# TravisWheelerLab/HAVAC

Measured on AMD Instinct MI355X. Metric: GCUPS (billion SSV cells/s); hit-list bit-exact vs softSsv, higher is better.
Workload: dtype i16

## Files before the change

havac_amd/csrc/ssv_kernels.hip.h:

```cpp
#pragma once
#include <hip/hip_runtime.h>
#include <stdint.h>
#include <utility>

namespace havac {

constexpr int kDiagsPerLane = 32;
constexpr int kRegs = kDiagsPerLane / 2;
constexpr int kTileDiags = 64 * kDiagsPerLane;
constexpr int kChunkRows = 32;
constexpr int kChunkPairs = kChunkRows / 2;
#ifndef HAVAC_BATCH
#define HAVAC_BATCH 8
#endif
#ifndef HAVAC_WAVES_PER_SIMD
#define HAVAC_WAVES_PER_SIMD 6
#endif
#ifndef HAVAC_WAVES_PER_BLOCK
#define HAVAC_WAVES_PER_BLOCK 4
#endif
constexpr int kWavesPerBlock = HAVAC_WAVES_PER_BLOCK;
constexpr int kModelSlack = 40;
constexpr uint32_t kScoreZero = 0x80008000u;
constexpr uint32_t kCrossedBits = 0x00010001u;
constexpr uint32_t kOutsideReset = 0x80008000u;
constexpr uint32_t kOutsideNeutral = 0u;
constexpr uint32_t kPadRow = 0u;
constexpr int kMaxRowCuts = 32;
constexpr int kMaxWalkRounds = 8;
constexpr int kWindowSteps = 4;

constexpr int kPairStride = 17 * 8;
constexpr uint32_t kOutsideCode = 16 * 8;
constexpr int kTableBytes = 2304;
constexpr int kHitStage = 128;
constexpr int kTailSlots = 128;
constexpr int kTicketStride = 16;
constexpr int kTicketCounters = 8;

__device__ __forceinline__ uint64_t hit_key(uint32_t row, uint64_t column, uint32_t row_bits) {
    const uint32_t seg = (uint32_t)(column >> 12) / 3u;
    const uint32_t in_seg = (uint32_t)column - seg * 12288u;
    return ((uint64_t)seg << (14 + row_bits)) | ((uint64_t)row << 14) | in_seg;
}

__device__ __forceinline__ uint64_t key_to_record(uint64_t key, uint32_t row_bits) {
    uint64_t in_seg = key & 0x3fffull;
    uint64_t row = (key >> 14) & ((1ull << row_bits) - 1ull);
    uint64_t seg = key >> (14 + row_bits);
    return in_seg | (seg << 14) | (row << 40);
}
__device__ __forceinline__ uint64_t record_to_key(uint64_t rec, uint32_t row_bits) {
    uint64_t in_seg = rec & 0x3fffull;
    uint64_t seg = (rec >> 14) & 0x3ffffffull;
    uint64_t row = rec >> 40;
    return (seg << (14 + row_bits)) | (row << 14) | in_seg;
}

__device__ __forceinline__ uint32_t padded_model_row(const uint32_t* __restrict__ phmm_rows, uint32_t nrows, uint32_t i) {
    return (i >= 1 && i <= nrows) ? phmm_rows[i - 1] : kPadRow;
}

__global__ void ssv_prepare_model(const int8_t* __restrict__ phmm, uint32_t nrows, uint32_t* __restrict__ rows, uint32_t nwords,
                                  uint32_t nrows_padded, uint32_t* __restrict__ flags, uint32_t nflagwords ,
                                  unsigned long long* __restrict__ hit_count, uint32_t* __restrict__ control, uint32_t ncontrol,
                                  uint32_t* __restrict__ handoff, uint32_t nhandoff) {
    const uint32_t* const phmm_rows = reinterpret_cast<const uint32_t*>(phmm);
    const uint32_t i = blockIdx.x * blockDim.x + threadIdx.x;
    if (i == 0) *hit_count = 0ull;
    if (i < ncontrol) control[i] = 0u;
    for (uint32_t k = i; k < nhandoff; k += gridDim.x * blockDim.x) handoff[k] = 0u;
    if (i < nwords) rows[i] = padded_model_row(phmm_rows, nrows, i);
    if (nflagwords == 0) return;
    const uint32_t chunk = i;
    const uint32_t p0 = chunk * kChunkRows;
    if (chunk / 4 >= nflagwords) return;
    uint32_t bits = 0;
    if (p0 < nrows_padded + kChunkRows) {
        int lowest[kChunkRows + 3];
#pragma unroll
        for (int k = 0; k < kChunkRows + 3; k++) {
            const uint32_t r = padded_model_row(phmm_rows, nrows, p0 + 1 + k);
            int m = 0;
#pragma unroll
            for (int a = 0; a < 4; a++) m = min(m, (int)(int8_t)(r >> (8 * a)));
            lowest[k] = m;
        }
#pragma unroll
        for (int q = 0; q < kChunkRows / kWindowSteps; q++) {
            const int high = lowest[4 * q] + lowest[4 * q + 1] + lowest[4 * q + 2], low = lowest[4 * q + 1] + lowest[4 * q + 2] + lowest[4 * q + 3];
            if (high >= -255 && low >= -255) bits |= 1u << q;
        }
    }
    reinterpret_cast<uint8_t*>(flags)[chunk] = (uint8_t)bits;
}

__global__ void ssv_pack_chars(const uint8_t* __restrict__ chars, uint64_t first_column, uint64_t nchars,
                               uint64_t ncolumns, uint32_t* __restrict__ packed) {
    const uint64_t word = first_column / 16 + (uint64_t)blockIdx.x * blockDim.x + threadIdx.x;
    const uint64_t column = word * 16;
    if (column >= ncolumns) return;
    uint32_t out = 0;
    if (column + 16 <= nchars) {
        const uint4 v = *reinterpret_cast<const uint4*>(chars + (column - first_column));
        const uint32_t w[4] = {v.x, v.y, v.z, v.w};
#pragma unroll
        for (int k = 0; k < 4; k++) {
            uint32_t t = (w[k] >> 1) & 0x03030303u;
            t ^= (t >> 1) & 0x01010101u;
            const uint32_t byte = (t | (t >> 6) | (t >> 12) | (t >> 18)) & 0xffu;
            out |= byte << (8 * k);
        }
    } else {
        for (int i = 0; i < 16; i++) {
            if (column + i >= nchars) break;
            uint32_t t = (chars[column - first_column + i] >> 1) & 3u;
            t ^= t >> 1;
            out |= t << (2 * i);
        }
    }
    packed[word] = out;
}

__global__ void ssv_patch_symbols(const uint64_t* __restrict__ columns, const uint8_t* __restrict__ symbols,
                                  uint64_t npatches, uint32_t* __restrict__ packed) {
    const uint64_t i = (uint64_t)blockIdx.x * blockDim.x + threadIdx.x;
    if (i >= npatches) return;
    const uint64_t column = columns[i];
    const uint32_t shift = (uint32_t)(column % 16) * 2;
    atomicAnd(&packed[column / 16], ~(3u << shift));
    atomicOr(&packed[column / 16], (uint32_t)(symbols[i] & 3u) << shift);
}

__global__ void ssv_pack_records(const uint8_t* __restrict__ chars, const uint64_t* __restrict__ out_start,
                                 const uint64_t* __restrict__ src_begin, const uint64_t* __restrict__ len, uint32_t nrecords,
                                 uint64_t layout_end, uint64_t ncolumns, uint32_t* __restrict__ packed, uint8_t* __restrict__ mask) {
    const uint64_t word = (uint64_t)blockIdx.x * blockDim.x + threadIdx.x;
    const uint64_t col0 = word * 16;
    if (col0 >= ncolumns) return;
    uint32_t lo = 0, hi = nrecords;
    while (lo < hi) {
        const uint32_t mid = (lo + hi) / 2;
        if (out_start[mid] <= col0) lo = mid + 1; else hi = mid;
    }
    uint32_t j = lo ? lo - 1 : 0;
    uint32_t out = 0, bits = 0;
    for (int i = 0; i < 16; i++) {
        const uint64_t col = col0 + i;
        while (j + 1 < nrecords && out_start[j + 1] <= col) j++;
        if (nrecords && col >= out_start[j]) {
            const uint64_t off = col - out_start[j];
            if (off < len[j]) {
                const uint32_t ch = chars[src_begin[j] + off] | 0x20u;
                const uint32_t code = ch == 'a' ? 0u : ch == 'c' ? 1u : ch == 'g' ? 2u : 3u;
                out |= code << (2 * i);
            }
            const uint64_t behind = out_start[j] + len[j];
            if ((i & 1) == 0 && col == behind + (behind & 1)) bits |= 1u << (i / 2);
        }
        if ((i & 1) == 0 && col >= layout_end) bits |= 1u << (i / 2);
    }
    packed[word] = out;
    mask[word] = (uint8_t)bits;
}

__global__ void ssv_reverse_strand(uint32_t* __restrict__ packed, uint64_t nf, const uint64_t* __restrict__ starts,
                                   const uint64_t* __restrict__ residues, uint32_t nrecords) {
    const uint64_t word = (uint64_t)blockIdx.x * blockDim.x + threadIdx.x;
    const uint64_t col0 = word * 16;
    if (col0 >= nf) return;
    auto symbol = [&](uint64_t col) -> uint32_t { return (packed[col / 16] >> (2 * (col % 16))) & 3u; };
    uint32_t lo = 0, hi = nrecords;
    while (lo < hi) {
        const uint32_t mid = (lo + hi) / 2;
        if (starts[mid] <= col0) lo = mid + 1; else hi = mid;
    }
    uint32_t j = lo ? lo - 1 : 0;
    uint32_t out = 0;
    for (int i = 0; i < 16; i++) {
        const uint64_t col = col0 + i;
        while (j + 1 < nrecords && starts[j + 1] <= col) j++;
        uint32_t code = symbol(col);
        if (nrecords && col >= starts[j] && col - starts[j] < residues[j])
            code = 3u - symbol(starts[j] + residues[j] - 1 - (col - starts[j]));
        out |= code << (2 * i);
    }
    packed[(nf + col0) / 16] = out;
}

typedef short short2v __attribute__((ext_vector_type(2)));
typedef uint32_t u32x2 __attribute__((ext_vector_type(2)));
typedef const __attribute__((address_space(3))) u32x2* lds_words_t;
typedef __attribute__((address_space(3))) u32x2* lds_words_out_t;

struct __attribute__((aligned(128))) WaveLds {
    uint8_t table[kTableBytes];
    uint64_t stage[kHitStage];
};

struct CellRecord {
    uint8_t prev;
    int8_t match;
    uint8_t score;
    uint8_t hit;
    uint8_t symbol;
    uint8_t pending;
    uint8_t zero;
    uint8_t written;
};

struct SsvRare {
    uint64_t* hits;
    unsigned long long* hit_count;
    uint64_t hit_capacity;
    int64_t col_begin;
    uint64_t col_span;
    const uint32_t* abort_flag;
    const uint16_t* pair_mask;
    uint32_t* tickets;
    uint32_t* block_flags;
    uint32_t* block_state;
    uint32_t* fault;
    uint32_t row_bits;
    int64_t first_diag; uint32_t tile_begin, ntiles;
    int64_t col_end;
    uint32_t parts_log2;
    uint32_t part_begin[9];
    uint32_t tiles_per_item;
    uint32_t single_tiles;
    uint32_t walk_slots, walk_rounds, walk_len[kMaxWalkRounds], walk_base[kMaxWalkRounds];
    uint32_t half_tail;
    uint32_t split_units;
    uint32_t nrow_blocks;
    uint32_t ncuts, uniform_rows;
    uint32_t row_cut[kMaxRowCuts + 1];
    uint64_t* tails; uint32_t* tail_counts;
    struct CellRecord* cells; int64_t cell_col0; uint32_t cell_row0, cell_rows, cell_cols;
};
typedef const __attribute__((address_space(4))) SsvRare* rare_args_t;
__device__ __forceinline__ rare_args_t rare_args() {
    rare_args_t p = (rare_args_t)__builtin_amdgcn_kernarg_segment_ptr();
    asm volatile("" : "+s"(p));
    return p;
}

struct HitSink {
    uint64_t* stage;
};

__device__ __forceinline__ uint64_t staged_to_key(uint64_t staged_record, uint32_t row_bits) {
    return hit_key((uint32_t)(staged_record >> 40), staged_record & ((1ull << 40) - 1ull), row_bits);
}

__device__ __forceinline__ uint32_t flush_hits(const HitSink& sink, const rare_args_t rare, uint32_t staged) {
    if (staged == 0) return 0;
    const uint32_t lane = __lane_id();
    uint64_t* const hits = rare->hits;
    const uint64_t capacity = rare->hit_capacity;
    const uint32_t row_bits = rare->row_bits;
    __builtin_amdgcn_fence(__ATOMIC_ACQ_REL, "wavefront");
    unsigned long long base = 0;
    if (lane == 0) base = atomicAdd(rare->hit_count, (unsigned long long)staged);
    const uint32_t lo = __builtin_amdgcn_readfirstlane((uint32_t)base);
    const uint32_t hi = __builtin_amdgcn_readfirstlane((uint32_t)(base >> 32));
    base = ((unsigned long long)hi << 32) | lo;
    for (uint32_t i = lane; i < staged; i += 64) {
        const unsigned long long idx = base + i;
        if (idx < capacity) hits[idx] = staged_to_key(sink.stage[i], row_bits);
    }
    __builtin_amdgcn_fence(__ATOMIC_ACQ_REL, "wavefront");
    return 0;
}

__device__ __noinline__ uint32_t flush_full(const HitSink sink, const rare_args_t rare, uint32_t staged) {
    return flush_hits(sink, rare, __builtin_amdgcn_readfirstlane(staged));
}

__device__ __forceinline__ int32_t scalar_sat_add(int32_t a, int32_t b) {
    const int32_t saturated = (b >> 31) ^ INT32_MAX;
    int32_t d;
    asm("s_add_i32 %0, %1, %2\n\ts_cselect_b32 %0, %3, %0" : "=&s"(d) : "s"(a), "s"(b), "s"(saturated) : "scc");
    return d;
}

struct ShardColumns { rare_args_t rare; int64_t begin; uint64_t span; };
__device__ __forceinline__ uint32_t emit_cell(const HitSink& sink, const ShardColumns& own, uint32_t staged, uint32_t row, int64_t column) {
    const rare_args_t rare = own.rare;
    if ((uint64_t)(column - own.begin) < own.span) {
        const uint64_t record = ((uint64_t)row << 40) | (uint64_t)column;
        const uint32_t addr = (uint32_t)(uintptr_t)(__attribute__((address_space(3))) uint64_t*)sink.stage + staged * 8;
        uint64_t saved_exec;
        asm volatile("s_mov_b64 %0, exec\n\ts_mov_b64 exec, 1\n\tds_write_b64 %1, %2\n\ts_mov_b64 exec, %0"
                     : "=&s"(saved_exec) : "v"(addr), "v"(record) : "memory");
        staged++;
        if (staged == kHitStage) staged = flush_full(sink, rare, staged);
    }
    return staged;
}

template <int P>
__device__ __forceinline__ u32x2 match_words(uint32_t code_addr, int extra = 0) {
    return *(lds_words_t)(uintptr_t)(code_addr + P * kPairStride + extra);
}
template <bool Resident>
__device__ __forceinline__ constexpr int slid_offset(int entry_index) { return Resident && entry_index < 16 ? kTableBytes : 0; }

__device__ __forceinline__ uint32_t opaque_uniform(uint32_t x) {
    x = __builtin_amdgcn_readfirstlane(x);
    asm("" : "+s"(x));
    return x;
}
__device__ __forceinline__ uint32_t fresh_uniform(uint32_t x) { asm volatile("" : "+s"(x)); return x; }
__device__ __forceinline__ int32_t clamp_to_4096(int64_t v) {
    const int32_t hi = (int32_t)opaque_uniform((uint32_t)((uint64_t)v >> 32));
    const uint32_t lo = opaque_uniform((uint32_t)v);
    return hi < 0 ? 0 : ((hi > 0 || lo > 4096u) ? 4096 : (int32_t)lo);
}

__device__ __forceinline__ uint32_t fresh_lane() {
    uint32_t lane;
    asm volatile("v_mbcnt_lo_u32_b32 %0, -1, 0\n\tv_mbcnt_hi_u32_b32 %0, -1, %0" : "=v"(lane));
    return lane;
}
struct LaneWords { uint32_t sel_second, entries, row_offset, lane8; };
__device__ __forceinline__ LaneWords read_lane_words(uint32_t lds_address) {
    LaneWords w;
    asm volatile("s_mov_b32 m0, %4\n\ts_nop 0\n\t"
                 "ds_read_addtid_b32 %0 offset:0\n\tds_read_addtid_b32 %1 offset:256\n\t"
                 "ds_read_addtid_b32 %2 offset:512\n\tds_read_addtid_b32 %3 offset:768\n\t"
                 "s_waitcnt lgkmcnt(0)"
                 : "=v"(w.sel_second), "=v"(w.entries), "=v"(w.row_offset), "=v"(w.lane8) : "s"(lds_address) : "m0", "memory");
    return w;
}

constexpr uint32_t kFlagSpecial = 2u;
constexpr int kFlagSafeShift = 8;
struct LazySymbols {
    uint32_t even[2], odd[2];
    uint32_t separators;
    uint32_t table_base;
    uint32_t special;
    int32_t valid_lo, valid_hi;
};

__device__ __forceinline__ void prepare_symbols(LazySymbols& z, uint32_t lo, uint32_t hi) {
    z.even[0] = (lo << 3) & 0x78787878u; z.odd[0] = (lo >> 1) & 0x78787878u;
    z.even[1] = (hi << 3) & 0x78787878u; z.odd[1] = (hi >> 1) & 0x78787878u;
}

template <int BYTE>
__device__ __forceinline__ uint32_t or_byte(uint32_t base, uint32_t word) {
    uint32_t out;
    if constexpr (BYTE == 0) asm("v_or_b32_sdwa %0, %1, %2 dst_sel:DWORD dst_unused:UNUSED_PAD src0_sel:DWORD src1_sel:BYTE_0" : "=v"(out) : "s"(base), "v"(word));
    if constexpr (BYTE == 1) asm("v_or_b32_sdwa %0, %1, %2 dst_sel:DWORD dst_unused:UNUSED_PAD src0_sel:DWORD src1_sel:BYTE_1" : "=v"(out) : "s"(base), "v"(word));
    if constexpr (BYTE == 2) asm("v_or_b32_sdwa %0, %1, %2 dst_sel:DWORD dst_unused:UNUSED_PAD src0_sel:DWORD src1_sel:BYTE_2" : "=v"(out) : "s"(base), "v"(word));
    if constexpr (BYTE == 3) asm("v_or_b32_sdwa %0, %1, %2 dst_sel:DWORD dst_unused:UNUSED_PAD src0_sel:DWORD src1_sel:BYTE_3" : "=v"(out) : "s"(base), "v"(word));
    return out;
}

template <int K>
__device__ __forceinline__ void expand_entry(uint32_t (&C)[32], const LazySymbols& z) {
    constexpr int n = K & 7;
    uint32_t entry = or_byte<n / 2>(z.table_base, (n & 1) ? z.odd[K / 8] : z.even[K / 8]);
    if (fresh_uniform(z.special) & kFlagSpecial) {
        const uint32_t lane32 = fresh_lane() * 32u;
        const int32_t q = (int32_t)lane32 + 2 * K;
        if (q < z.valid_lo || q >= z.valid_hi || ((z.separators >> K) & 1u)) entry = z.table_base + kOutsideCode;
    }
    C[16 + K] = entry;
}

template <int Q>
__device__ __forceinline__ void expand_for_window(uint32_t (&C)[32], const LazySymbols& z) {
    if constexpr (Q == 0) {
        expand_entry<0>(C, z);
    } else {
        expand_entry<2 * Q - 1>(C, z);
        expand_entry<2 * Q>(C, z);
    }
}

template <int... K>
__device__ __forceinline__ void expand_all(uint32_t (&C)[32], const LazySymbols& z, std::integer_sequence<int, K...>) {
    (expand_entry<K>(C, z), ...);
}

struct TraceWindow { CellRecord* cells; int64_t col0; uint32_t row0, nrows, ncols; };
__device__ __noinline__ void trace_cells_of_step(TraceWindow win, uint32_t second_of_pair, uint32_t reg, uint32_t t, int64_t wave_diag0,
                                                 uint32_t before, uint32_t mword, uint32_t after, uint32_t code) {
    const int64_t column = wave_diag0 + (int64_t)(32u * __lane_id() + 2u * reg) + (int64_t)t;
    const uint64_t dc = (uint64_t)(column - win.col0);
    const uint8_t symbol = code > 15u ? 0xffu : (uint8_t)(second_of_pair ? code >> 2 : code & 3u);
    for (uint32_t half = 0; half < 2; half++) {
        const uint32_t dr = t - half - win.row0;
        if (dr < win.nrows && dc < (uint64_t)win.ncols) {
            const uint32_t b = (before >> (16 * half)) & 0xffffu, a = (after >> (16 * half)) & 0xffffu;
            CellRecord rec;
            rec.pending = (b & 0xffu) != 0;
            rec.hit = !rec.pending && (a & 0xffu) != 0;
            rec.prev = rec.pending ? 0 : (uint8_t)((b ^ 0x8000u) >> 8);
            rec.score = (rec.pending || rec.hit) ? 0 : (uint8_t)((a ^ 0x8000u) >> 8);
            rec.match = (int8_t)(uint8_t)(mword >> (8 + 16 * half));
            rec.symbol = symbol;
            rec.zero = 0;
            rec.written = 1;
            win.cells[(size_t)dr * win.ncols + (size_t)dc] = rec;
        }
    }
}
__device__ __forceinline__ TraceWindow trace_window() {
    const rare_args_t rare = rare_args();
    return TraceWindow{rare->cells, rare->cell_col0, rare->cell_row0, rare->cell_rows, rare->cell_cols};
}
template <bool SecondOfPair>
__device__ __forceinline__ void trace_step(const TraceWindow& win, uint32_t reg, uint32_t t, int64_t wave_diag0, uint32_t before,
                                           uint32_t mword, uint32_t after, uint32_t entry, uint32_t table_base) {
    trace_cells_of_step(win, SecondOfPair ? 1u : 0u, reg, t, wave_diag0, before, mword, after, (entry - table_base) >> 3);
}

template <int Q, int I>
__device__ __forceinline__ void window_inputs(uint32_t l, const uint32_t (&cur)[kRegs], const uint32_t (&nxt)[kRegs],
                                              const uint32_t (&C)[32], uint32_t& s, uint32_t& now, uint32_t& entry0,
                                              uint32_t& entry1) {
    asm volatile("v_readlane_b32 %0, %4, %8\n\tv_readlane_b32 %1, %5, %8\n\tv_readlane_b32 %2, %6, %8\n\tv_readlane_b32 %3, %7, %8"
                 : "=&s"(s), "=&s"(now), "=&s"(entry0), "=&s"(entry1)
                 : "v"(cur[I]), "v"(nxt[I]), "v"(C[2 * Q + I]), "v"(C[2 * Q + 1 + I]), "s"(l));
}

__device__ __forceinline__ void write_score_lane(uint32_t (&n)[kRegs], uint32_t s, uint32_t l, uint32_t r) {
    static_assert(kRegs == 16, "the asm below names sixteen registers");
    asm volatile("s_mov_b32 m0, %[l]\n\t"
                 "s_cmp_ge_u32 %[r], 8\n\ts_cbranch_scc1 .Lhavac_w8_16_%=\n\t"
                 "s_cmp_ge_u32 %[r], 4\n\ts_cbranch_scc1 .Lhavac_w4_8_%=\n\t"
                 "s_cmp_ge_u32 %[r], 2\n\ts_cbranch_scc1 .Lhavac_w2_4_%=\n\t"
                 "s_cmp_ge_u32 %[r], 1\n\ts_cbranch_scc1 .Lhavac_w1_2_%=\n\t"
                 "v_writelane_b32 %0, %[s], m0\n\ts_branch .Lhavac_wend_%=\n"
                 ".Lhavac_w1_2_%=:\n\t"
                 "v_writelane_b32 %1, %[s], m0\n\ts_branch .Lhavac_wend_%=\n"
                 ".Lhavac_w2_4_%=:\n\t"
                 "s_cmp_ge_u32 %[r], 3\n\ts_cbranch_scc1 .Lhavac_w3_4_%=\n\t"
                 "v_writelane_b32 %2, %[s], m0\n\ts_branch .Lhavac_wend_%=\n"
                 ".Lhavac_w3_4_%=:\n\t"
                 "v_writelane_b32 %3, %[s], m0\n\ts_branch .Lhavac_wend_%=\n"
                 ".Lhavac_w4_8_%=:\n\t"
                 "s_cmp_ge_u32 %[r], 6\n\ts_cbranch_scc1 .Lhavac_w6_8_%=\n\t"
                 "s_cmp_ge_u32 %[r], 5\n\ts_cbranch_scc1 .Lhavac_w5_6_%=\n\t"
                 "v_writelane_b32 %4, %[s], m0\n\ts_branch .Lhavac_wend_%=\n"
                 ".Lhavac_w5_6_%=:\n\t"
                 "v_writelane_b32 %5, %[s], m0\n\ts_branch .Lhavac_wend_%=\n"
                 ".Lhavac_w6_8_%=:\n\t"
                 "s_cmp_ge_u32 %[r], 7\n\ts_cbranch_scc1 .Lhavac_w7_8_%=\n\t"
                 "v_writelane_b32 %6, %[s], m0\n\ts_branch .Lhavac_wend_%=\n"
                 ".Lhavac_w7_8_%=:\n\t"
                 "v_writelane_b32 %7, %[s], m0\n\ts_branch .Lhavac_wend_%=\n"
                 ".Lhavac_w8_16_%=:\n\t"
                 "s_cmp_ge_u32 %[r], 12\n\ts_cbranch_scc1 .Lhavac_w12_16_%=\n\t"
                 "s_cmp_ge_u32 %[r], 10\n\ts_cbranch_scc1 .Lhavac_w10_12_%=\n\t"
                 "s_cmp_ge_u32 %[r], 9\n\ts_cbranch_scc1 .Lhavac_w9_10_%=\n\t"
                 "v_writelane_b32 %8, %[s], m0\n\ts_branch .Lhavac_wend_%=\n"
                 ".Lhavac_w9_10_%=:\n\t"
                 "v_writelane_b32 %9, %[s], m0\n\ts_branch .Lhavac_wend_%=\n"
                 ".Lhavac_w10_12_%=:\n\t"
                 "s_cmp_ge_u32 %[r], 11\n\ts_cbranch_scc1 .Lhavac_w11_12_%=\n\t"
                 "v_writelane_b32 %10, %[s], m0\n\ts_branch .Lhavac_wend_%=\n"
                 ".Lhavac_w11_12_%=:\n\t"
                 "v_writelane_b32 %11, %[s], m0\n\ts_branch .Lhavac_wend_%=\n"
                 ".Lhavac_w12_16_%=:\n\t"
                 "s_cmp_ge_u32 %[r], 14\n\ts_cbranch_scc1 .Lhavac_w14_16_%=\n\t"
                 "s_cmp_ge_u32 %[r], 13\n\ts_cbranch_scc1 .Lhavac_w13_14_%=\n\t"
                 "v_writelane_b32 %12, %[s], m0\n\ts_branch .Lhavac_wend_%=\n"
                 ".Lhavac_w13_14_%=:\n\t"
                 "v_writelane_b32 %13, %[s], m0\n\ts_branch .Lhavac_wend_%=\n"
                 ".Lhavac_w14_16_%=:\n\t"
                 "s_cmp_ge_u32 %[r], 15\n\ts_cbranch_scc1 .Lhavac_w15_16_%=\n\t"
                 "v_writelane_b32 %14, %[s], m0\n\ts_branch .Lhavac_wend_%=\n"
                 ".Lhavac_w15_16_%=:\n\t"
                 "v_writelane_b32 %15, %[s], m0\n\ts_branch .Lhavac_wend_%=\n"
                 ".Lhavac_wend_%=:"
                 : "+v"(n[0]), "+v"(n[1]), "+v"(n[2]), "+v"(n[3]), "+v"(n[4]), "+v"(n[5]), "+v"(n[6]), "+v"(n[7]),
                   "+v"(n[8]), "+v"(n[9]), "+v"(n[10]), "+v"(n[11]), "+v"(n[12]), "+v"(n[13]), "+v"(n[14]), "+v"(n[15])
                 : [s] "s"(s), [l] "s"(l), [r] "s"(r)
                 : "m0", "scc");
}

template <int Q, int Lo, int Hi>
__device__ __forceinline__ void find_marked(uint32_t l, const uint32_t (&cur)[kRegs], const uint32_t (&nxt)[kRegs],
                                            const uint32_t (&C)[32], uint32_t& r, uint32_t& s, uint32_t& now,
                                            uint32_t& entry0, uint32_t& entry1) {
    if constexpr (Hi - Lo == 1) {
        r = Lo;
        window_inputs<Q, Lo>(l, cur, nxt, C, s, now, entry0, entry1);
    } else {
        constexpr int Mid = (Lo + Hi) / 2;
        uint32_t lower = nxt[Lo];
#pragma unroll
        for (int i = Lo + 1; i < Mid; i++) lower |= nxt[i];
        if (__builtin_amdgcn_readlane(lower, l) & kCrossedBits) find_marked<Q, Lo, Mid>(l, cur, nxt, C, r, s, now, entry0, entry1);
        else find_marked<Q, Mid, Hi>(l, cur, nxt, C, r, s, now, entry0, entry1);
    }
}

#ifdef HAVAC_SLOW_CLOCKS
__device__ unsigned long long g_slow_clocks[4];
__shared__ unsigned long long s_slow_clocks[4];
#endif
template <bool Resident, int Q, int NSTEPS, int... I>
__device__ __forceinline__ void window_slow(const uint32_t (&cur)[kRegs], uint32_t (&nxt)[kRegs], const uint32_t (&C)[32],
                                            unsigned long long lanes, int report_from, const HitSink& sink, uint32_t& staged,
                                            uint32_t step0, int64_t wave_diag0, std::integer_sequence<int, I...>) {
#if defined(HAVAC_SLOW_CLOCKS) && HAVAC_SLOW_CLOCKS > 1
    const uint64_t slow_t0 = __builtin_readcyclecounter();
#endif
    ShardColumns own;
    own.rare = rare_args();
    own.begin = own.rare->col_begin;
    own.span = own.rare->col_span;
    do {
        do {
            const uint32_t l = (uint32_t)__builtin_ctzll(lanes);
            lanes &= lanes - 1;
            uint32_t r = 0, s = 0, now = 0, entry0 = 0, entry1 = 0;
            find_marked<Q, 0, kRegs>(l, cur, nxt, C, r, s, now, entry0, entry1);
            uint32_t w[kWindowSteps] = {0, 0, 0, 0};
            if constexpr (Resident) {
                entry0 += 2 * Q + r < 16 ? (uint32_t)kTableBytes : 0u;
                entry1 += 2 * Q + 1 + r < 16 ? (uint32_t)kTableBytes : 0u;
            }
            const u32x2 wa = match_words<2 * Q>(entry0);
            w[0] = (uint32_t)__builtin_amdgcn_readfirstlane(wa.x);
            w[1] = (uint32_t)__builtin_amdgcn_readfirstlane(wa.y);
            if constexpr (NSTEPS > 2) {
                const u32x2 wb = match_words<2 * Q + 1>(entry1);
                w[2] = (uint32_t)__builtin_amdgcn_readfirstlane(wb.x);
                w[3] = (uint32_t)__builtin_amdgcn_readfirstlane(wb.y);
            }
            const uint32_t t0 = step0 + kWindowSteps * Q;
            const int64_t column0 = wave_diag0 + (int64_t)(32 * l + 2 * r) + (int64_t)t0;
            int32_t low = (int32_t)(s << 16), high = (int32_t)(s & 0xffff0000u);
            uint32_t crossed = 0;
            if (now & 1u) {
#pragma unroll
                for (int k = 0; k < NSTEPS; k++) {
                    low = scalar_sat_add(low, (int32_t)(w[k] << 16));
                    const bool hit = low == INT32_MAX;
                    crossed |= hit ? (1u << k) : 0u;
                    low = hit ? INT32_MIN : low;
                }
                now = (now & 0xffff0000u) | ((uint32_t)low >> 16);
            }
            if (now & 0x10000u) {
#pragma unroll
                for (int k = 0; k < NSTEPS; k++) {
                    high = scalar_sat_add(high, (int32_t)(w[k] & 0xffff0000u));
                    const bool hit = high == INT32_MAX;
                    crossed |= hit ? (16u << k) : 0u;
                    high = hit ? INT32_MIN : high;
                }
                now = (now & 0xffffu) | ((uint32_t)high & 0xffff0000u);
            }
            crossed &= ((0xfu << report_from) & 0xfu) * 0x11u;
            while (crossed) {
                const uint32_t bit = (uint32_t)__builtin_ctz(crossed);
                crossed &= crossed - 1;
                const uint32_t k = bit & 3u, behind = bit >> 2;
                staged = emit_cell(sink, own, staged, t0 + k - behind, column0 + k);
            }
            s = now;
            write_score_lane(nxt, s, l, r);
        } while (lanes);
        uint32_t marked = 0;
#pragma unroll
        for (int i = 0; i < kRegs; i++) marked |= nxt[i];
        lanes = __ballot((marked & kCrossedBits) != 0);
    } while (lanes);
#if defined(HAVAC_SLOW_CLOCKS) && HAVAC_SLOW_CLOCKS > 1
    if (fresh_lane() == 0) { atomicAdd(&s_slow_clocks[0], (unsigned long long)(__builtin_readcyclecounter() - slow_t0)); atomicAdd(&s_slow_clocks[1], 1ull); }
#endif
}

template <bool Trace, bool Resident, int Q, int... I>
__device__ __forceinline__ void step_window(const uint32_t (&cur)[kRegs], uint32_t (&nxt)[kRegs], const uint32_t (&C)[32],
                                            uint32_t safe, const HitSink& sink, uint32_t& staged, uint32_t step0,
                                            int64_t wave_diag0, uint32_t table_base, std::integer_sequence<int, I...> regs) {
    static_assert(sizeof...(I) == kRegs, "one index per score register");
    constexpr int H = HAVAC_BATCH;
    constexpr int NB = kRegs / H;
    TraceWindow win{};
    if constexpr (Trace) win = trace_window();
#pragma unroll
    for (int h = 0; h < NB; h++) {
        u32x2 m[H];
        __builtin_amdgcn_sched_barrier(0);
#pragma unroll
        for (int i = 0; i < H; i++) m[i] = match_words<2 * Q>(C[2 * Q + h * H + i], slid_offset<Resident>(2 * Q + h * H + i));
        __builtin_amdgcn_sched_barrier(0);
#pragma unroll
        for (int i = 0; i < H; i++) asm("v_pk_add_i16 %0, %1, %2 clamp" : "=v"(nxt[h * H + i]) : "v"(cur[h * H + i]), "v"(m[i].x));
        if constexpr (Trace) {
#pragma unroll
            for (int i = 0; i < H; i++)
                trace_step<false>(win, h * H + i, step0 + 4 * Q, wave_diag0, cur[h * H + i], m[i].x, nxt[h * H + i], C[2 * Q + h * H + i], table_base);
        }
        uint32_t mid[H];
        if constexpr (Trace) {
#pragma unroll
            for (int i = 0; i < H; i++) mid[i] = nxt[h * H + i];
        }
#pragma unroll
        for (int i = 0; i < H; i++) asm("v_pk_add_i16 %0, %0, %1 clamp" : "+v"(nxt[h * H + i]) : "v"(m[i].y));
        if constexpr (Trace) {
#pragma unroll
            for (int i = 0; i < H; i++)
                trace_step<true>(win, h * H + i, step0 + 4 * Q + 1, wave_diag0, mid[i], m[i].y, nxt[h * H + i], C[2 * Q + h * H + i], table_base);
        }
    }
    if (!(fresh_uniform(safe) & (1u << (kFlagSafeShift + Q)))) {
        uint32_t any = 0;
#pragma unroll
        for (int i = 0; i < kRegs; i++) any |= nxt[i];
        if (const unsigned long long lanes = __ballot((any & kCrossedBits) != 0); __builtin_expect(lanes != 0, 0))
            window_slow<Resident, Q, 2>(cur, nxt, C, lanes, 0, sink, staged, step0, wave_diag0, regs);
    }
#pragma unroll
    for (int h = 0; h < NB; h++) {
        u32x2 m[H];
        __builtin_amdgcn_sched_barrier(0);
#pragma unroll
        for (int i = 0; i < H; i++) m[i] = match_words<2 * Q + 1>(C[2 * Q + 1 + h * H + i], slid_offset<Resident>(2 * Q + 1 + h * H + i));
        __builtin_amdgcn_sched_barrier(0);
        uint32_t mid[H];
        if constexpr (Trace) {
#pragma unroll
            for (int i = 0; i < H; i++) mid[i] = nxt[h * H + i];
        }
#pragma unroll
        for (int i = 0; i < H; i++) asm("v_pk_add_i16 %0, %0, %1 clamp" : "+v"(nxt[h * H + i]) : "v"(m[i].x));
        if constexpr (Trace) {
#pragma unroll
            for (int i = 0; i < H; i++) {
                trace_step<false>(win, h * H + i, step0 + 4 * Q + 2, wave_diag0, mid[i], m[i].x, nxt[h * H + i], C[2 * Q + 1 + h * H + i], table_base);
                mid[i] = nxt[h * H + i];
            }
        }
#pragma unroll
        for (int i = 0; i < H; i++) asm("v_pk_add_i16 %0, %0, %1 clamp" : "+v"(nxt[h * H + i]) : "v"(m[i].y));
        if constexpr (Trace) {
#pragma unroll
            for (int i = 0; i < H; i++)
                trace_step<true>(win, h * H + i, step0 + 4 * Q + 3, wave_diag0, mid[i], m[i].y, nxt[h * H + i], C[2 * Q + 1 + h * H + i], table_base);
        }
    }
    uint32_t any = 0;
#pragma unroll
    for (int i = 0; i < kRegs; i++) any |= nxt[i];
    if (const unsigned long long lanes = __ballot((any & kCrossedBits) != 0); __builtin_expect(lanes != 0, 0))
        window_slow<Resident, Q, kWindowSteps>(cur, nxt, C, lanes, (int)(2u - 2u * ((safe >> (kFlagSafeShift + Q)) & 1u)), sink, staged, step0, wave_diag0, regs);
}

template <bool Trace, bool Resident, int PQ, int... I>
__device__ __forceinline__ void step_last(const uint32_t (&cur)[kRegs], uint32_t (&nxt)[kRegs], const uint32_t (&C)[32],
                                          const HitSink& sink, uint32_t& staged, uint32_t step0, int64_t wave_diag0,
                                          uint32_t table_base, std::integer_sequence<int, I...> regs) {
    constexpr int H = kRegs / 2;
    TraceWindow win{};
    if constexpr (Trace) win = trace_window();
#pragma unroll
    for (int h = 0; h < 2; h++) {
        u32x2 m[H];
        __builtin_amdgcn_sched_barrier(0);
#pragma unroll
        for (int i = 0; i < H; i++) m[i] = match_words<2 * PQ>(C[2 * PQ + h * H + i], slid_offset<Resident>(2 * PQ + h * H + i));
        __builtin_amdgcn_sched_barrier(0);
#pragma unroll
        for (int i = 0; i < H; i++) asm("v_pk_add_i16 %0, %1, %2 clamp" : "=v"(nxt[h * H + i]) : "v"(cur[h * H + i]), "v"(m[i].x));
        if constexpr (Trace) {
#pragma unroll
            for (int i = 0; i < H; i++)
                trace_step<false>(win, h * H + i, step0 + kWindowSteps * PQ, wave_diag0, cur[h * H + i], m[i].x, nxt[h * H + i], C[2 * PQ + h * H + i], table_base);
        }
    }
    uint32_t any = 0;
#pragma unroll
    for (int i = 0; i < kRegs; i++) any |= nxt[i];
    if (const unsigned long long lanes = __ballot((any & kCrossedBits) != 0); __builtin_expect(lanes != 0, 0))
        window_slow<Resident, PQ, 1>(cur, nxt, C, lanes, 0, sink, staged, step0, wave_diag0, regs);
}

template <bool Trace, bool Resident, int... Q>
__device__ __forceinline__ void step_windows(uint32_t (&a)[kRegs], uint32_t (&b)[kRegs], uint32_t (&C)[32],
                                             const LazySymbols& z, uint32_t safe, const HitSink& sink, uint32_t& staged,
                                             uint32_t step0, int64_t wave_diag0, std::integer_sequence<int, Q...>) {
    static_assert(sizeof...(Q) % 2 == 0 && sizeof...(Q) * kWindowSteps <= kChunkRows, "an even number of windows");
    constexpr int last = std::max({Q...});
    ((expand_for_window<Q>(C, z),
      (Q % 2 == 0 ? step_window<Trace, Resident, Q>(a, b, C, safe, sink, staged, step0, wave_diag0, z.table_base, std::make_integer_sequence<int, kRegs>{})
                  : step_window<Trace, Resident, Q>(b, a, C, safe, sink, staged, step0, wave_diag0, z.table_base, std::make_integer_sequence<int, kRegs>{}))), ...);
    if constexpr (last == kChunkRows / kWindowSteps - 1) expand_entry<15>(C, z);
}

__device__ __forceinline__ void leave_block(const uint64_t* const stage, const uint32_t staged, const uint32_t wave) {
#ifdef HAVAC_SLOW_CLOCKS
    __syncthreads();
    if (threadIdx.x == 0) {
        if (s_slow_clocks[1]) { atomicAdd(&g_slow_clocks[0], s_slow_clocks[0]); atomicAdd(&g_slow_clocks[1], s_slow_clocks[1]); }
        atomicAdd(&g_slow_clocks[2], (unsigned long long)__builtin_readcyclecounter() - s_slow_clocks[2]);
        atomicAdd(&g_slow_clocks[3], (unsigned long long)wall_clock64() - s_slow_clocks[3]);
    }
#endif
    __shared__ uint32_t block_staged[kWavesPerBlock];
    __shared__ unsigned long long block_base;
    const uint32_t lane_again = __lane_id();
    if (lane_again == 0) block_staged[wave] = staged;
    __syncthreads();
    uint32_t total = 0, before_me = 0;
#pragma unroll
    for (int w = 0; w < kWavesPerBlock; w++) { total += block_staged[w]; before_me += (uint32_t)w < wave ? block_staged[w] : 0u; }
    const rare_args_t rare = rare_args();
    uint64_t* const tails = rare->tails;
    if (tails && total <= (uint32_t)kTailSlots) {
        if (wave == 0 && lane_again == 0) rare->tail_counts[blockIdx.x] = total;
        if (staged) {
            const uint32_t row_bits = rare->row_bits;
            uint64_t* const mine = tails + (size_t)blockIdx.x * kTailSlots + before_me;
            for (uint32_t i = lane_again; i < staged; i += 64) mine[i] = staged_to_key(stage[i], row_bits);
        }
        return;
    }
    if (wave == 0 && lane_again == 0) {
        if (tails) rare->tail_counts[blockIdx.x] = 0;
        block_base = total ? atomicAdd(rare->hit_count, (unsigned long long)total) : 0ull;
    }
    __syncthreads();
    if (staged) {
        uint64_t* const hits = rare->hits;
        const uint64_t capacity = rare->hit_capacity;
        const uint32_t row_bits = rare->row_bits;
        const unsigned long long base = block_base + before_me;
        for (uint32_t i = lane_again; i < staged; i += 64)
            if (base + i < capacity) hits[base + i] = staged_to_key(stage[i], row_bits);
    }
}

__device__ __forceinline__ uint32_t word_selector(uint32_t a) { return 0x040c000cu + a * 0x01000100u; }

constexpr uint32_t kWholeTile = 0xffffffffu;
constexpr int kBlocksPerCu = 4 * HAVAC_WAVES_PER_SIMD / kWavesPerBlock;
constexpr uint32_t kHandoffSpins = 1u << 26;

template <bool Trace>
__device__ __forceinline__ void ssv_diag_body(const uint8_t* __restrict__ seq, const uint32_t* __restrict__ rows,
                                              const uint32_t* __restrict__ safe_chunks, const int64_t nsymbols,
                                              const uint32_t nrows_padded) {
    __shared__ WaveLds wave_lds[kWavesPerBlock];
#ifdef HAVAC_SLOW_CLOCKS
    if (threadIdx.x == 0) { s_slow_clocks[0] = s_slow_clocks[1] = 0; s_slow_clocks[2] = __builtin_readcyclecounter(); s_slow_clocks[3] = wall_clock64(); }
    __syncthreads();
#endif

    const uint32_t lane = threadIdx.x & 63;
    const uint32_t has_mask = opaque_uniform(rare_args()->pair_mask != nullptr ? 1u : 0u);
    const uint32_t wave = __builtin_amdgcn_readfirstlane(threadIdx.x >> 6);
    WaveLds* const lds = &wave_lds[wave];
    const HitSink sink{lds->stage};
    uint32_t staged = 0;

    const uint32_t table_base = __builtin_amdgcn_readfirstlane((uint32_t)(uintptr_t)(__attribute__((address_space(3))) uint8_t*)lds->table);
    const uint32_t my_pair = lane >> 2, my_b = lane & 3;
    __shared__ uint32_t lane_words[4][64];
    lane_words[0][lane] = word_selector(my_b);
    lane_words[1][lane] = my_pair * kPairStride + my_b * 32;
    lane_words[2][lane] = my_pair * 8;
    lane_words[3][lane] = lane * 8;
    const uint32_t lane_words_address = __builtin_amdgcn_readfirstlane((uint32_t)(uintptr_t)(__attribute__((address_space(3))) uint32_t*)&lane_words[0][0]);
    if (my_b == 0) {
        const uint32_t outside = has_mask ? kOutsideReset : kOutsideNeutral;
        *(lds_words_out_t)(uintptr_t)(table_base + my_pair * kPairStride + kOutsideCode) = u32x2{outside, outside};
    }

    auto run_item = [&](const uint32_t tile_arg, const uint32_t block_arg ,
                        const uint32_t slot_arg ) -> bool {
        const uint32_t tile_in_launch = __builtin_amdgcn_readfirstlane(tile_arg), block = __builtin_amdgcn_readfirstlane(block_arg);
        const uint32_t handoff_slot = __builtin_amdgcn_readfirstlane(slot_arg);
        const uint32_t cut = block != kWholeTile ? 1u : 0u;
        const rare_args_t launch = rare_args();
        const uint32_t tile = launch->tile_begin + tile_in_launch;
        const int64_t d0 = launch->first_diag + (int64_t)tile * kTileDiags;
        int64_t lo64 = -d0 - kTileDiags;
        if (lo64 < 0) lo64 = 0;
        if (lo64 > (int64_t)nrows_padded) lo64 = nrows_padded;
        int64_t hi64 = launch->col_end - d0;
        if (hi64 > (int64_t)nrows_padded) hi64 = nrows_padded;
        if (hi64 < 0) hi64 = 0;
        const uint32_t p_lo = __builtin_amdgcn_readfirstlane((uint32_t)lo64), p_hi = __builtin_amdgcn_readfirstlane((uint32_t)hi64);
        uint32_t p_begin = p_lo, p_end = p_hi;
        if (cut) {
            const uint32_t ncuts = launch->ncuts, uniform_rows = launch->uniform_rows, last_cut = launch->row_cut[ncuts];
            const uint32_t b0 = block < ncuts ? launch->row_cut[block] : last_cut + (block - ncuts) * uniform_rows;
            const uint32_t b1 = block < ncuts ? launch->row_cut[block + 1] : last_cut + (block - ncuts + 1) * uniform_rows;
            if (p_begin < b0) p_begin = b0;
            if (p_end > b1) p_end = b1;
        }
        if (p_begin >= p_end) return true;
        uint32_t abort_now = 0;
        {
            const uint32_t* const abort_flag = rare_args()->abort_flag;
            if (abort_flag) abort_now = __hip_atomic_load(abort_flag, __ATOMIC_RELAXED, __HIP_MEMORY_SCOPE_SYSTEM);
        }

        uint32_t x[kRegs], x2[kRegs];
        if (p_begin > p_lo) {
            const rare_args_t rare = rare_args();
            const uint32_t* const abort_flag = rare->abort_flag;
            uint32_t* const block_flags = rare->block_flags;
            uint32_t* const fault = rare->fault;
            const uint32_t* const tile_state = rare->block_state + (size_t)handoff_slot * (kRegs / 2 * 64);
            uint32_t spins = 0;
            while (__hip_atomic_load(block_flags + handoff_slot, __ATOMIC_RELAXED, __HIP_MEMORY_SCOPE_AGENT) < block) {
                __builtin_amdgcn_s_sleep(32);
                ++spins;
                if ((spins & 63u) == 0) {
                    if (abort_flag && __hip_atomic_load(abort_flag, __ATOMIC_RELAXED, __HIP_MEMORY_SCOPE_SYSTEM) != 0) return false;
                    if (__hip_atomic_load(fault, __ATOMIC_RELAXED, __HIP_MEMORY_SCOPE_AGENT) != 0) return false;
                }
                if (spins == kHandoffSpins) {
                    if (fresh_lane() == 0) __hip_atomic_store(fault, 1u, __ATOMIC_RELAXED, __HIP_MEMORY_SCOPE_AGENT);
                    return false;
                }
            }
            __builtin_amdgcn_fence(__ATOMIC_ACQUIRE, "agent");
            const uint32_t my_lane = fresh_lane();
#pragma unroll
            for (int i = 0; i < kRegs / 2; i++) {
                const uint32_t packed = tile_state[i * 64 + my_lane];
                x[2 * i] = __builtin_amdgcn_perm(0u, packed, 0x010c000cu);
                x[2 * i + 1] = __builtin_amdgcn_perm(0u, packed, 0x030c020cu);
            }
        } else {
#pragma unroll
// ... 426 lines not shown
```

Baseline: 57530.

## Vectorize slow-path threshold replay across lanes instead of per-lane scalar loop

The rare slow path that replays a window after a score crosses threshold used to walk marked lanes one at a time, reading each lane's state into scalars and doing saturating scalar adds. It now selects a marked register wave-wide by ballot and replays the window steps with packed vector adds for all lanes at once. Crossings are recorded as bits in the score register, and only lanes with report bits are scanned to emit hits. It also adds an option to inline the hit flush. The aim is to cut the serial per-lane cost when many lanes cross; the risk is extra vector work and subtle bit-exactness bugs in the crossing and report encoding.

```diff
diff --git a/havac_amd/csrc/ssv_kernels.hip.h b/havac_amd/csrc/ssv_kernels.hip.h
--- a/havac_amd/csrc/ssv_kernels.hip.h
+++ b/havac_amd/csrc/ssv_kernels.hip.h
@@ -23,6 +23,7 @@
 constexpr int kModelSlack = 40;
 constexpr uint32_t kScoreZero = 0x80008000u;
 constexpr uint32_t kCrossedBits = 0x00010001u;
+constexpr uint32_t kReportBits = 0x000f000fu;
 constexpr uint32_t kOutsideReset = 0x80008000u;
 constexpr uint32_t kOutsideNeutral = 0u;
 constexpr uint32_t kPadRow = 0u;
@@ -276,14 +277,8 @@
     return flush_hits(sink, rare, __builtin_amdgcn_readfirstlane(staged));
 }
 
-__device__ __forceinline__ int32_t scalar_sat_add(int32_t a, int32_t b) {
-    const int32_t saturated = (b >> 31) ^ INT32_MAX;
-    int32_t d;
-    asm("s_add_i32 %0, %1, %2\n\ts_cselect_b32 %0, %3, %0" : "=&s"(d) : "s"(a), "s"(b), "s"(saturated) : "scc");
-    return d;
-}
-
 struct ShardColumns { rare_args_t rare; int64_t begin; uint64_t span; };
+template <bool InlineFlush = false>
 __device__ __forceinline__ uint32_t emit_cell(const HitSink& sink, const ShardColumns& own, uint32_t staged, uint32_t row, int64_t column) {
     const rare_args_t rare = own.rare;
     if ((uint64_t)(column - own.begin) < own.span) {
@@ -293,7 +288,7 @@
         asm volatile("s_mov_b64 %0, exec\n\ts_mov_b64 exec, 1\n\tds_write_b64 %1, %2\n\ts_mov_b64 exec, %0"
                      : "=&s"(saved_exec) : "v"(addr), "v"(record) : "memory");
         staged++;
-        if (staged == kHitStage) staged = flush_full(sink, rare, staged);
+        if (staged == kHitStage) staged = InlineFlush ? flush_hits(sink, rare, kHitStage) : flush_full(sink, rare, staged);
     }
     return staged;
 }
@@ -418,85 +413,84 @@
     trace_cells_of_step(win, SecondOfPair ? 1u : 0u, reg, t, wave_diag0, before, mword, after, (entry - table_base) >> 3);
 }
 
-template <int Q, int I>
-__device__ __forceinline__ void window_inputs(uint32_t l, const uint32_t (&cur)[kRegs], const uint32_t (&nxt)[kRegs],
-                                              const uint32_t (&C)[32], uint32_t& s, uint32_t& now, uint32_t& entry0,
-                                              uint32_t& entry1) {
-    asm volatile("v_readlane_b32 %0, %4, %8\n\tv_readlane_b32 %1, %5, %8\n\tv_readlane_b32 %2, %6, %8\n\tv_readlane_b32 %3, %7, %8"
-                 : "=&s"(s), "=&s"(now), "=&s"(entry0), "=&s"(entry1)
-                 : "v"(cur[I]), "v"(nxt[I]), "v"(C[2 * Q + I]), "v"(C[2 * Q + 1 + I]), "s"(l));
-}
-
-__device__ __forceinline__ void write_score_lane(uint32_t (&n)[kRegs], uint32_t s, uint32_t l, uint32_t r) {
+template <int Q, int I, bool Four>
+__device__ __forceinline__ void register_inputs(const uint32_t (&cur)[kRegs], const uint32_t (&C)[32], uint32_t& s,
+                                                uint32_t& entry0, uint32_t& entry1) {
+    if constexpr (Four)
+        asm volatile("v_mov_b32 %0, %3\n\tv_mov_b32 %1, %4\n\tv_mov_b32 %2, %5"
+                     : "=&v"(s), "=&v"(entry0), "=&v"(entry1) : "v"(cur[I]), "v"(C[2 * Q + I]), "v"(C[2 * Q + 1 + I]));
+    else
+        asm volatile("v_mov_b32 %0, %2\n\tv_mov_b32 %1, %3" : "=&v"(s), "=&v"(entry0) : "v"(cur[I]), "v"(C[2 * Q + I]));
+}
+
+__device__ __forceinline__ void write_score_register(uint32_t (&n)[kRegs], uint32_t x, uint32_t r) {
     static_assert(kRegs == 16, "the asm below names sixteen registers");
-    asm volatile("s_mov_b32 m0, %[l]\n\t"
-                 "s_cmp_ge_u32 %[r], 8\n\ts_cbranch_scc1 .Lhavac_w8_16_%=\n\t"
+    asm volatile("s_cmp_ge_u32 %[r], 8\n\ts_cbranch_scc1 .Lhavac_w8_16_%=\n\t"
                  "s_cmp_ge_u32 %[r], 4\n\ts_cbranch_scc1 .Lhavac_w4_8_%=\n\t"
                  "s_cmp_ge_u32 %[r], 2\n\ts_cbranch_scc1 .Lhavac_w2_4_%=\n\t"
                  "s_cmp_ge_u32 %[r], 1\n\ts_cbranch_scc1 .Lhavac_w1_2_%=\n\t"
-                 "v_writelane_b32 %0, %[s], m0\n\ts_branch .Lhavac_wend_%=\n"
+                 "v_and_b32 %0, 0xff00ff00, %[x]\n\ts_branch .Lhavac_wend_%=\n"
                  ".Lhavac_w1_2_%=:\n\t"
-                 "v_writelane_b32 %1, %[s], m0\n\ts_branch .Lhavac_wend_%=\n"
+                 "v_and_b32 %1, 0xff00ff00, %[x]\n\ts_branch .Lhavac_wend_%=\n"
                  ".Lhavac_w2_4_%=:\n\t"
                  "s_cmp_ge_u32 %[r], 3\n\ts_cbranch_scc1 .Lhavac_w3_4_%=\n\t"
-                 "v_writelane_b32 %2, %[s], m0\n\ts_branch .Lhavac_wend_%=\n"
+                 "v_and_b32 %2, 0xff00ff00, %[x]\n\ts_branch .Lhavac_wend_%=\n"
                  ".Lhavac_w3_4_%=:\n\t"
-                 "v_writelane_b32 %3, %[s], m0\n\ts_branch .Lhavac_wend_%=\n"
+                 "v_and_b32 %3, 0xff00ff00, %[x]\n\ts_branch .Lhavac_wend_%=\n"
                  ".Lhavac_w4_8_%=:\n\t"
                  "s_cmp_ge_u32 %[r], 6\n\ts_cbranch_scc1 .Lhavac_w6_8_%=\n\t"
                  "s_cmp_ge_u32 %[r], 5\n\ts_cbranch_scc1 .Lhavac_w5_6_%=\n\t"
-                 "v_writelane_b32 %4, %[s], m0\n\ts_branch .Lhavac_wend_%=\n"
+                 "v_and_b32 %4, 0xff00ff00, %[x]\n\ts_branch .Lhavac_wend_%=\n"
                  ".Lhavac_w5_6_%=:\n\t"
-                 "v_writelane_b32 %5, %[s], m0\n\ts_branch .Lhavac_wend_%=\n"
+                 "v_and_b32 %5, 0xff00ff00, %[x]\n\ts_branch .Lhavac_wend_%=\n"
                  ".Lhavac_w6_8_%=:\n\t"
                  "s_cmp_ge_u32 %[r], 7\n\ts_cbranch_scc1 .Lhavac_w7_8_%=\n\t"
-                 "v_writelane_b32 %6, %[s], m0\n\ts_branch .Lhavac_wend_%=\n"
+                 "v_and_b32 %6, 0xff00ff00, %[x]\n\ts_branch .Lhavac_wend_%=\n"
                  ".Lhavac_w7_8_%=:\n\t"
-                 "v_writelane_b32 %7, %[s], m0\n\ts_branch .Lhavac_wend_%=\n"
+                 "v_and_b32 %7, 0xff00ff00, %[x]\n\ts_branch .Lhavac_wend_%=\n"
                  ".Lhavac_w8_16_%=:\n\t"
                  "s_cmp_ge_u32 %[r], 12\n\ts_cbranch_scc1 .Lhavac_w12_16_%=\n\t"
                  "s_cmp_ge_u32 %[r], 10\n\ts_cbranch_scc1 .Lhavac_w10_12_%=\n\t"
                  "s_cmp_ge_u32 %[r], 9\n\ts_cbranch_scc1 .Lhavac_w9_10_%=\n\t"
-                 "v_writelane_b32 %8, %[s], m0\n\ts_branch .Lhavac_wend_%=\n"
+                 "v_and_b32 %8, 0xff00ff00, %[x]\n\ts_branch .Lhavac_wend_%=\n"
                  ".Lhavac_w9_10_%=:\n\t"
-                 "v_writelane_b32 %9, %[s], m0\n\ts_branch .Lhavac_wend_%=\n"
+                 "v_and_b32 %9, 0xff00ff00, %[x]\n\ts_branch .Lhavac_wend_%=\n"
                  ".Lhavac_w10_12_%=:\n\t"
                  "s_cmp_ge_u32 %[r], 11\n\ts_cbranch_scc1 .Lhavac_w11_12_%=\n\t"
-                 "v_writelane_b32 %10, %[s], m0\n\ts_branch .Lhavac_wend_%=\n"
+                 "v_and_b32 %10, 0xff00ff00, %[x]\n\ts_branch .Lhavac_wend_%=\n"
                  ".Lhavac_w11_12_%=:\n\t"
-                 "v_writelane_b32 %11, %[s], m0\n\ts_branch .Lhavac_wend_%=\n"
+                 "v_and_b32 %11, 0xff00ff00, %[x]\n\ts_branch .Lhavac_wend_%=\n"
                  ".Lhavac_w12_16_%=:\n\t"
                  "s_cmp_ge_u32 %[r], 14\n\ts_cbranch_scc1 .Lhavac_w14_16_%=\n\t"
                  "s_cmp_ge_u32 %[r], 13\n\ts_cbranch_scc1 .Lhavac_w13_14_%=\n\t"
-                 "v_writelane_b32 %12, %[s], m0\n\ts_branch .Lhavac_wend_%=\n"
+                 "v_and_b32 %12, 0xff00ff00, %[x]\n\ts_branch .Lhavac_wend_%=\n"
                  ".Lhavac_w13_14_%=:\n\t"
-                 "v_writelane_b32 %13, %[s], m0\n\ts_branch .Lhavac_wend_%=\n"
+                 "v_and_b32 %13, 0xff00ff00, %[x]\n\ts_branch .Lhavac_wend_%=\n"
                  ".Lhavac_w14_16_%=:\n\t"
                  "s_cmp_ge_u32 %[r], 15\n\ts_cbranch_scc1 .Lhavac_w15_16_%=\n\t"
-                 "v_writelane_b32 %14, %[s], m0\n\ts_branch .Lhavac_wend_%=\n"
+                 "v_and_b32 %14, 0xff00ff00, %[x]\n\ts_branch .Lhavac_wend_%=\n"
                  ".Lhavac_w15_16_%=:\n\t"
-                 "v_writelane_b32 %15, %[s], m0\n\ts_branch .Lhavac_wend_%=\n"
+                 "v_and_b32 %15, 0xff00ff00, %[x]\n\ts_branch .Lhavac_wend_%=\n"
                  ".Lhavac_wend_%=:"
                  : "+v"(n[0]), "+v"(n[1]), "+v"(n[2]), "+v"(n[3]), "+v"(n[4]), "+v"(n[5]), "+v"(n[6]), "+v"(n[7]),
                    "+v"(n[8]), "+v"(n[9]), "+v"(n[10]), "+v"(n[11]), "+v"(n[12]), "+v"(n[13]), "+v"(n[14]), "+v"(n[15])
-                 : [s] "s"(s), [l] "s"(l), [r] "s"(r)
-                 : "m0", "scc");
-}
-
-template <int Q, int Lo, int Hi>
-__device__ __forceinline__ void find_marked(uint32_t l, const uint32_t (&cur)[kRegs], const uint32_t (&nxt)[kRegs],
-                                            const uint32_t (&C)[32], uint32_t& r, uint32_t& s, uint32_t& now,
-                                            uint32_t& entry0, uint32_t& entry1) {
+                 : [x] "v"(x), [r] "s"(r)
+                 : "scc");
+}
+
+template <int Q, bool Four, int Lo, int Hi>
+__device__ __forceinline__ void find_marked(const uint32_t (&cur)[kRegs], const uint32_t (&nxt)[kRegs], const uint32_t (&C)[32],
+                                            uint32_t& r, uint32_t& s, uint32_t& entry0, uint32_t& entry1) {
     if constexpr (Hi - Lo == 1) {
         r = Lo;
-        window_inputs<Q, Lo>(l, cur, nxt, C, s, now, entry0, entry1);
+        register_inputs<Q, Lo, Four>(cur, C, s, entry0, entry1);
     } else {
         constexpr int Mid = (Lo + Hi) / 2;
         uint32_t lower = nxt[Lo];
 #pragma unroll
         for (int i = Lo + 1; i < Mid; i++) lower |= nxt[i];
-        if (__builtin_amdgcn_readlane(lower, l) & kCrossedBits) find_marked<Q, Lo, Mid>(l, cur, nxt, C, r, s, now, entry0, entry1);
-        else find_marked<Q, Mid, Hi>(l, cur, nxt, C, r, s, now, entry0, entry1);
+        if (__ballot((lower & kCrossedBits) != 0)) find_marked<Q, Four, Lo, Mid>(cur, nxt, C, r, s, entry0, entry1);
+        else find_marked<Q, Four, Mid, Hi>(cur, nxt, C, r, s, entry0, entry1);
     }
 }
 
@@ -506,73 +500,56 @@
 #endif
 template <bool Resident, int Q, int NSTEPS, int... I>
 __device__ __forceinline__ void window_slow(const uint32_t (&cur)[kRegs], uint32_t (&nxt)[kRegs], const uint32_t (&C)[32],
-                                            unsigned long long lanes, int report_from, const HitSink& sink, uint32_t& staged,
-                                            uint32_t step0, int64_t wave_diag0, std::integer_sequence<int, I...>) {
+                                            int report_from, const HitSink& sink, uint32_t& staged, uint32_t step0,
+                                            int64_t wave_diag0, std::integer_sequence<int, I...>) {
 #if defined(HAVAC_SLOW_CLOCKS) && HAVAC_SLOW_CLOCKS > 1
     const uint64_t slow_t0 = __builtin_readcyclecounter();
 #endif
+    constexpr bool Four = NSTEPS > 2;
     ShardColumns own;
     own.rare = rare_args();
     own.begin = own.rare->col_begin;
     own.span = own.rare->col_span;
+    const uint32_t t0 = step0 + kWindowSteps * Q;
+    uint32_t marked;
     do {
-        do {
+        uint32_t r = 0, x = 0, entry0 = 0, entry1 = 0;
+        find_marked<Q, Four, 0, kRegs>(cur, nxt, C, r, x, entry0, entry1);
+        if constexpr (Resident) {
+            entry0 += 2 * Q + r < 16 ? (uint32_t)kTableBytes : 0u;
+            if constexpr (Four) entry1 += 2 * Q + 1 + r < 16 ? (uint32_t)kTableBytes : 0u;
+        }
+        const u32x2 wa = match_words<2 * Q>(entry0);
+        u32x2 wb = {0u, 0u};
+        if constexpr (Four) wb = match_words<2 * Q + 1>(entry1);
+        const uint32_t w[kWindowSteps] = {wa.x, wa.y, wb.x, wb.y};
+        uint32_t crossed = 0;
+#pragma unroll
+        for (int k = 0; k < NSTEPS; k++) {
+            asm("v_pk_add_i16 %0, %0, %1 clamp" : "+v"(x) : "v"(w[k]));
+            const uint32_t c = x & kCrossedBits;
+            asm("v_pk_add_u16 %0, %0, %1" : "+v"(x) : "v"(c));
+            crossed |= c << k;
+        }
+        x |= crossed & ((0xfu << report_from) & 0xfu) * 0x10001u;
+        write_score_register(nxt, x, r);
+        unsigned long long lanes = __ballot((x & kReportBits) != 0);
+        const int64_t column0 = wave_diag0 + (int64_t)(2 * r + t0);
+        while (lanes) {
             const uint32_t l = (uint32_t)__builtin_ctzll(lanes);
             lanes &= lanes - 1;
-            uint32_t r = 0, s = 0, now = 0, entry0 = 0, entry1 = 0;
-            find_marked<Q, 0, kRegs>(l, cur, nxt, C, r, s, now, entry0, entry1);
-            uint32_t w[kWindowSteps] = {0, 0, 0, 0};
-            if constexpr (Resident) {
-                entry0 += 2 * Q + r < 16 ? (uint32_t)kTableBytes : 0u;
-                entry1 += 2 * Q + 1 + r < 16 ? (uint32_t)kTableBytes : 0u;
+            uint32_t bits = __builtin_amdgcn_readlane(x, l) & kReportBits;
+            while (bits) {
+                const uint32_t bit = (uint32_t)__builtin_ctz(bits);
+                bits &= bits - 1;
+                const uint32_t k = bit & 15u, behind = bit >> 4;
+                staged = emit_cell<Resident>(sink, own, staged, t0 + k - behind, column0 + (int64_t)(32 * l + k));
             }
-            const u32x2 wa = match_words<2 * Q>(entry0);
-            w[0] = (uint32_t)__builtin_amdgcn_readfirstlane(wa.x);
-            w[1] = (uint32_t)__builtin_amdgcn_readfirstlane(wa.y);
-            if constexpr (NSTEPS > 2) {
-                const u32x2 wb = match_words<2 * Q + 1>(entry1);
-                w[2] = (uint32_t)__builtin_amdgcn_readfirstlane(wb.x);
-                w[3] = (uint32_t)__builtin_amdgcn_readfirstlane(wb.y);
-            }
-            const uint32_t t0 = step0 + kWindowSteps * Q;
-            const int64_t column0 = wave_diag0 + (int64_t)(32 * l + 2 * r) + (int64_t)t0;
-            int32_t low = (int32_t)(s << 16), high = (int32_t)(s & 0xffff0000u);
-            uint32_t crossed = 0;
-            if (now & 1u) {
-#pragma unroll
-                for (int k = 0; k < NSTEPS; k++) {
-                    low = scalar_sat_add(low, (int32_t)(w[k] << 16));
-                    const bool hit = low == INT32_MAX;
-                    crossed |= hit ? (1u << k) : 0u;
-                    low = hit ? INT32_MIN : low;
-                }
-                now = (now & 0xffff0000u) | ((uint32_t)low >> 16);
-            }
-            if (now & 0x10000u) {
-#pragma unroll
-                for (int k = 0; k < NSTEPS; k++) {
-                    high = scalar_sat_add(high, (int32_t)(w[k] & 0xffff0000u));
-                    const bool hit = high == INT32_MAX;
-                    crossed |= hit ? (16u << k) : 0u;
-                    high = hit ? INT32_MIN : high;
-                }
-                now = (now & 0xffffu) | ((uint32_t)high & 0xffff0000u);
-            }
-            crossed &= ((0xfu << report_from) & 0xfu) * 0x11u;
-            while (crossed) {
-                const uint32_t bit = (uint32_t)__builtin_ctz(crossed);
-                crossed &= crossed - 1;
-                const uint32_t k = bit & 3u, behind = bit >> 2;
-                staged = emit_cell(sink, own, staged, t0 + k - behind, column0 + k);
-            }
-            s = now;
-            write_score_lane(nxt, s, l, r);
-        } while (lanes);
-        uint32_t marked = 0;
+        }
+        marked = 0;
 #pragma unroll
         for (int i = 0; i < kRegs; i++) marked |= nxt[i];
-        lanes = __ballot((marked & kCrossedBits) != 0);
-    } while (lanes);
+    } while (__ballot((marked & kCrossedBits) != 0));
 #if defined(HAVAC_SLOW_CLOCKS) && HAVAC_SLOW_CLOCKS > 1
     if (fresh_lane() == 0) { atomicAdd(&s_slow_clocks[0], (unsigned long long)(__builtin_readcyclecounter() - slow_t0)); atomicAdd(&s_slow_clocks[1], 1ull); }
 #endif
@@ -619,7 +596,7 @@
 #pragma unroll
         for (int i = 0; i < kRegs; i++) any |= nxt[i];
         if (const unsigned long long lanes = __ballot((any & kCrossedBits) != 0); __builtin_expect(lanes != 0, 0))
-            window_slow<Resident, Q, 2>(cur, nxt, C, lanes, 0, sink, staged, step0, wave_diag0, regs);
+            window_slow<Resident, Q, 2>(cur, nxt, C, 0, sink, staged, step0, wave_diag0, regs);
     }
 #pragma unroll
     for (int h = 0; h < NB; h++) {
@@ -654,7 +631,7 @@
 #pragma unroll
     for (int i = 0; i < kRegs; i++) any |= nxt[i];
     if (const unsigned long long lanes = __ballot((any & kCrossedBits) != 0); __builtin_expect(lanes != 0, 0))
-        window_slow<Resident, Q, kWindowSteps>(cur, nxt, C, lanes, (int)(2u - 2u * ((safe >> (kFlagSafeShift + Q)) & 1u)), sink, staged, step0, wave_diag0, regs);
+        window_slow<Resident, Q, kWindowSteps>(cur, nxt, C, (int)(2u - 2u * ((safe >> (kFlagSafeShift + Q)) & 1u)), sink, staged, step0, wave_diag0, regs);
 }
 
 template <bool Trace, bool Resident, int PQ, int... I>
@@ -683,7 +660,7 @@
 #pragma unroll
     for (int i = 0; i < kRegs; i++) any |= nxt[i];
     if (const unsigned long long lanes = __ballot((any & kCrossedBits) != 0); __builtin_expect(lanes != 0, 0))
-        window_slow<Resident, PQ, 1>(cur, nxt, C, lanes, 0, sink, staged, step0, wave_diag0, regs);
+        window_slow<Resident, PQ, 1>(cur, nxt, C, 0, sink, staged, step0, wave_diag0, regs);
 }
 
 template <bool Trace, bool Resident, int... Q>
```

New measurement: 57670, median of 6. No clear change (+0.3%).
